# prosysscience/JSSEnv

Hardware: AMD Instinct MI355X
Metric: env steps/sec (batched) (higher is better)
Workload: dtype int32

## Files before the change

__graft_entry__.py:

```python
import os
import sys

ROOT = os.path.dirname(os.path.abspath(__file__))
if ROOT not in sys.path:
    sys.path.insert(0, ROOT)


def build() -> None:
    from jssenv_amd.build import build_cpu_twin, build_extension
    path = build_extension(force=True)
    assert os.path.isfile(path)
    twin = build_cpu_twin(force=True)
    assert os.path.isfile(twin)
    from oracle import build_oracle
    build_oracle(force=True)
    import ctypes
    from jssenv_amd import _abi
    _abi.bind_keys(_abi.bind_rules(_abi.bind_search(_abi.bind(ctypes.CDLL(path)))))
    _abi.bind_keys(_abi.bind_rules(_abi.bind_search(_abi.bind(ctypes.CDLL(twin)))))
    _abi.bind_bound(ctypes.CDLL(_abi.library_path("libjss_bound_hip.so")))
    _abi.bind_bound(ctypes.CDLL(twin))
    _abi.bind_order(ctypes.CDLL(_abi.library_path("libjss_order_hip.so")))
    _abi.bind_order(ctypes.CDLL(twin))
    _abi.bind_tabu(ctypes.CDLL(_abi.library_path("libjss_tabu_hip.so")))
    _abi.bind_tabu(ctypes.CDLL(twin))
    _abi.bind_block(ctypes.CDLL(_abi.library_path("libjss_block_hip.so")))
    _abi.bind_block(ctypes.CDLL(twin))
    _abi.bind_relink(ctypes.CDLL(_abi.library_path("libjss_relink_hip.so")))
    _abi.bind_relink(ctypes.CDLL(twin))
    _abi.bind_decode(ctypes.CDLL(_abi.library_path("libjss_decode_hip.so")))
    _abi.bind_decode(ctypes.CDLL(twin))
    _abi.bind_machine(ctypes.CDLL(_abi.library_path("libjss_machine_hip.so")))
    _abi.bind_machine(ctypes.CDLL(twin))
    _abi.bind_carlier(ctypes.CDLL(_abi.library_path("libjss_carlier_hip.so")))
    _abi.bind_carlier(ctypes.CDLL(twin))
    _abi.bind_propagate(ctypes.CDLL(_abi.library_path("libjss_propagate_hip.so")))
    _abi.bind_propagate(ctypes.CDLL(twin))
    import jssenv_amd
    print(f"built {path} and {twin}")


def smoke() -> None:
    import numpy as np
    import torch
    assert torch.cuda.is_available(), "smoke() needs a GPU"
    from jssenv_amd import BatchedJssEnv, builtin_instance
    from oracle import OracleEnv

    inst = builtin_instance("ta01")
    B, seed = 256, 3
    env = BatchedJssEnv(inst, batch=B, device="cuda:0", seed=seed)
    env.reset()
# ... 24 lines not shown
```

jssenv_amd/_abi.py:

```python
from __future__ import annotations

import ctypes as C
import os
from typing import Optional

ABI_VERSION = 14
STATE_LAYOUT = 7
MAX_JOBS, MAX_MACHINES = 128, 64
F_TODO, F_CUR, F_LEFT, F_PERF, F_IDLE, F_IDLE_LAST, F_F4, F_NEXT, NF = 0, 1, 2, 3, 4, 5, 6, 7, 8
TODO_MASK, FLAG_LEGAL, FLAG_BLOCKED, NEXT2_SHIFT = 255, 256, 512, 10
FC_W0, FC_LEFT_F4, FC_IDLE, FC_IDLE_LAST, NFC = 0, 1, 2, 3, 4
FC_TODO_MASK, FC_FLAG_LEGAL, FC_FLAG_BLOCKED, FC_FLAG_F4_ONE, FC_PERF_SHIFT = 127, 128, 256, 512, 10
FM_W0, FM_LEFT_F4, FM_PERF_NEXT, FM_NEXT_NEXT2, FM_IDLE, FM_IDLE_LAST, NFM = 0, 1, 2, 3, 4, 5, 6
FM_TODO_MASK, FM_FLAG_LEGAL, FM_FLAG_BLOCKED, FM_FLAG_F4_ONE, FM_CUR_SHIFT, FM_OP_MASK = 63, 64, 128, 256, 9, 0x1FFFFF
H_CLOCK, H_EPISODE, H_STEP, H_STATUS = 0, 1, 2, 3
NH = 4
C_JOBS, C_MACHINES, C_MAX_TIME_OP, C_TABLE, C_MAX_TIME_JOBS, C_SUM_OP = 0, 1, 2, 3, 4, 5
C_RCP_MAX_TIME_OP, C_RCP_MAX_TIME_JOBS, C_RCP_SUM_OP, C_RCP_MACHINES, NC = 6, 7, 8, 9, 12
STATUS_NOOP = 256
F4_ONE = -1
I_JOBS, I_MACHINES, I_MAX_TIME_OP, I_MAX_TIME_JOBS, I_SUM_OP = 0, 1, 2, 3, 4
I_RCP_MAX_TIME_OP, I_RCP_MAX_TIME_JOBS, I_RCP_SUM_OP, I_RCP_MACHINES, NI = 5, 6, 7, 8, 12
ERR_ILLEGAL_ACTION, ERR_NOPE_IDLE, ERR_BAD_ACTION, ERR_BAD_LOGITS, ERR_BAD_INDEX = 1, 2, 4, 8, 16
ACTION_SKIP, ACTION_RESET, ACTION_CLOSE = -1, -2, -3
# ... 78 lines not shown
MACHINE_SYMBOLS = ("jss_machine_relax", "jss_bottleneck_build")
BOTTLENECK_NI = 4
BOTTLENECK_MAX_REOPT = 8

CARLIER_VERSION = 1
CARLIER_SYMBOLS = ("jss_machine_solve", "jss_bottleneck_exact")
CARLIER_MAX_NODES = 4096
CARLIER_MAX_DEPTH = 64
EXACT_NI = 8

PROPAGATE_VERSION = 1
PROPAGATE_SYMBOLS = ("jss_propagate",)
PROPAGATE_MAX_PASSES = 4096
PROPAGATE_MAX_TIME = 0x3FFFFFFF
PROPAGATE_FIXPOINT, PROPAGATE_REFUTED, PROPAGATE_BUDGET = 0, 1, 2

_p = C.c_void_p


class JssDesc(C.Structure):
    _fields_ = [("batch", C.c_int32), ("jmax", C.c_int32), ("mmax", C.c_int32), ("n_tables", C.c_int32),
                ("ops", _p), ("rem", _p), ("inst", _p), ("table_of_env", _p), ("env_ids", _p),
                ("env_id_base", C.c_int64), ("kernel", C.c_int32), ("threads", C.c_int32),
                ("jmin", C.c_int32), ("record_ints", C.c_int32), ("cr_factor", C.c_double),
                ("jclass", C.c_int32), ("mclass", C.c_int32)]


class JssState(C.Structure):
    _fields_ = [("env", _p), ("env_const", _p), ("job", _p), ("machine", _p), ("solution", _p), ("counters", _p)]

# ... 315 lines not shown
    symbols, binder, header = _FAMILIES[family]
    first = getattr(lib, symbols[0], None)
    if first is not None and first.argtypes is not None:
        return lib
    if not all(hasattr(lib, name) for name in symbols):
        if what is None:
            return None
        raise RuntimeError(f"{what}: the loaded library does not export the {family}_* calls of include/{header}")
    return binder(lib)


def check(lib, rc: int, what: str):
    if rc != 0:
        msg = lib.jss_error_string(rc)
        raise RuntimeError(f"{what} failed: {rc} ({msg.decode() if msg else '?'})")
```

jssenv_amd/backends.py:

```python
from __future__ import annotations

import ctypes as C
import os

import numpy as np

from . import _abi


class HipBackend:

    name = "hip"
    default_kernel = "auto"

    def __init__(self, device=None):
        import torch
        if not torch.cuda.is_available():
            raise RuntimeError("jssenv_amd needs an AMD GPU (torch.cuda.is_available() is False); there is no silent "
                               "CPU fallback -- pass device='cpu' to run on the host-core twin (libjss_cpu.so) on purpose")
        path = _abi.library_path()
        if not os.path.isfile(path):
            raise RuntimeError(f"{path} is missing: build it with `python -c 'import __graft_entry__ as g; g.build()'`")
        self.torch = torch
        self.device = torch.device(device if device is not None else f"cuda:{torch.cuda.current_device()}")
# ... 7 lines not shown
        if not self.lib.jss_backend().startswith(b"hip"):
            raise RuntimeError(f"{path} is not the HIP library ({self.lib.jss_backend()!r})")
        self._scalars = {}
        self._stream_arrays = {}
        self._raw_stream = getattr(torch._C, "_cuda_getCurrentRawStream", None)
        self._beam_lib = None
        self._bound_lib = None
        self._order_lib = None
        self._tabu_lib = None
        self._block_lib = None
        self._relink_lib = None
        self._decode_lib = None
        self._machine_lib = None
        self._carlier_lib = None
        self._propagate_lib = None

    @property
    def beam_lib(self):
        if self._beam_lib is None:
            path = _abi.library_path("libjss_beam_hip.so")
            if not os.path.isfile(path):
                raise RuntimeError(f"{path} is missing: build it with `python -c 'import __graft_entry__ as g; g.build()'`")
            self._beam_lib = _abi.bind_beam(C.CDLL(path))
        return self._beam_lib

    @property
    def bound_lib(self):
        if self._bound_lib is None:
            path = _abi.library_path("libjss_bound_hip.so")
            if not os.path.isfile(path):
# ... 345 lines not shown
```

jssenv_amd/build.py:

```python
import os
import shutil
import subprocess

_HERE = os.path.dirname(os.path.abspath(__file__))
_ROOT = os.path.dirname(_HERE)
SRC = os.path.join(_HERE, "csrc", "jss_kernels.hip")
OUT = os.path.join(_HERE, "libjss_hip.so")
FLAGS = ["--offload-arch=gfx950", "-O3", "-std=c++17", "-fPIC", "-shared", "-I" + os.path.join(_ROOT, "include"),
         "-mllvm", "-amdgpu-atomic-optimizer-strategy=None"]
CPU_SRC = os.path.join(_HERE, "csrc", "jss_cpu.cpp")
CPU_OUT = os.path.join(_HERE, "libjss_cpu.so")
CPU_FLAGS = ["-O3", "-std=c++17", "-fopenmp", "-fPIC", "-shared", "-Wall", "-I" + os.path.join(_ROOT, "include")]
_HEADER = os.path.join(_ROOT, "include", "jss_hip.h")
_SEARCH = os.path.join(_ROOT, "include", "jss_search.h")
_RULES = os.path.join(_ROOT, "include", "jss_rules.h")
_KEYS = os.path.join(_ROOT, "include", "jss_keys.h")
_BEAM = os.path.join(_ROOT, "include", "jss_beam.h")
BEAM_SRC = os.path.join(_HERE, "csrc", "jss_beam.hip")
BEAM_OUT = os.path.join(_HERE, "libjss_beam_hip.so")
_BOUND = os.path.join(_ROOT, "include", "jss_bound.h")
BOUND_SRC = os.path.join(_HERE, "csrc", "jss_bound.hip")
BOUND_OUT = os.path.join(_HERE, "libjss_bound_hip.so")
_ORDER = os.path.join(_ROOT, "include", "jss_order.h")
ORDER_SRC = os.path.join(_HERE, "csrc", "jss_order.hip")
# ... 7 lines not shown
_RELINK = os.path.join(_ROOT, "include", "jss_relink.h")
RELINK_SRC = os.path.join(_HERE, "csrc", "jss_relink.hip")
RELINK_OUT = os.path.join(_HERE, "libjss_relink_hip.so")
_DECODE = os.path.join(_ROOT, "include", "jss_decode.h")
DECODE_SRC = os.path.join(_HERE, "csrc", "jss_decode.hip")
DECODE_OUT = os.path.join(_HERE, "libjss_decode_hip.so")
_MACHINE = os.path.join(_ROOT, "include", "jss_machine.h")
MACHINE_SRC = os.path.join(_HERE, "csrc", "jss_machine.hip")
MACHINE_OUT = os.path.join(_HERE, "libjss_machine_hip.so")
_CARLIER = os.path.join(_ROOT, "include", "jss_carlier.h")
CARLIER_SRC = os.path.join(_HERE, "csrc", "jss_carlier.hip")
CARLIER_OUT = os.path.join(_HERE, "libjss_carlier_hip.so")
_PROPAGATE = os.path.join(_ROOT, "include", "jss_propagate.h")
PROPAGATE_SRC = os.path.join(_HERE, "csrc", "jss_propagate.hip")
PROPAGATE_OUT = os.path.join(_HERE, "libjss_propagate_hip.so")
_OWN_LIBRARY = (os.path.basename(BEAM_SRC), os.path.basename(BOUND_SRC), os.path.basename(ORDER_SRC),
                os.path.basename(TABU_SRC), os.path.basename(BLOCK_SRC), os.path.basename(RELINK_SRC),
                os.path.basename(DECODE_SRC), os.path.basename(MACHINE_SRC), os.path.basename(CARLIER_SRC), os.path.basename(PROPAGATE_SRC))
_CHECKS = os.path.join(_HERE, "csrc", "jss_abi_checks.hpp")
_ROWS = os.path.join(_HERE, "csrc", "jss_env_rows.hpp")


def hipcc() -> str:
    for cand in (shutil.which("hipcc"), "/opt/rocm/bin/hipcc"):
        if cand and os.path.isfile(cand):
            return cand
    raise RuntimeError("hipcc not found")


def _fresh(out, deps):
    return os.path.isfile(out) and all(os.path.getmtime(out) >= os.path.getmtime(d) for d in deps)


def build_extension(force: bool = False, extra=(), out: str = OUT) -> str:
    csrc = os.path.dirname(SRC)
    deps = [os.path.join(csrc, f) for f in os.listdir(csrc) if f.endswith((".hip", ".hpp")) and f not in _OWN_LIBRARY] + [_HEADER, _SEARCH, _RULES, _KEYS, _BEAM, _BOUND, _ORDER, _TABU, _BLOCK, _RELINK, _DECODE, _MACHINE, _CARLIER, _PROPAGATE]
    if out == OUT:
        build_beam_extension(force)
        build_bound_extension(force)
        build_order_extension(force)
        build_tabu_extension(force)
        build_block_extension(force)
        build_relink_extension(force)
        build_decode_extension(force)
        build_machine_extension(force)
        build_carlier_extension(force)
        build_propagate_extension(force)
    if not force and _fresh(out, deps):
        return out
    subprocess.check_call([hipcc(), *FLAGS, *extra, SRC, "-o", out])
    return out


def build_beam_extension(force: bool = False) -> str:
    if not force and _fresh(BEAM_OUT, [BEAM_SRC, _CHECKS, _HEADER, _SEARCH, _RULES, _KEYS, _BEAM, _BOUND, _ORDER, _TABU, _BLOCK, _RELINK, _DECODE, _MACHINE, _CARLIER, _PROPAGATE]):
        return BEAM_OUT
    tmp = BEAM_OUT + f".tmp{os.getpid()}"
    subprocess.check_call([hipcc(), *FLAGS, BEAM_SRC, "-o", tmp])
    os.replace(tmp, BEAM_OUT)
    return BEAM_OUT


# ... 64 lines not shown
    if not force and _fresh(CARLIER_OUT, [CARLIER_SRC, _CHECKS, _HEADER, _SEARCH, _RULES, _KEYS, _BEAM, _BOUND, _ORDER, _TABU, _BLOCK, _RELINK, _DECODE, _MACHINE, _CARLIER, _PROPAGATE]):
        return CARLIER_OUT
    tmp = CARLIER_OUT + f".tmp{os.getpid()}"
    subprocess.check_call([hipcc(), *FLAGS, CARLIER_SRC, "-o", tmp])
    os.replace(tmp, CARLIER_OUT)
    return CARLIER_OUT


def build_propagate_extension(force: bool = False) -> str:
    if not force and _fresh(PROPAGATE_OUT, [PROPAGATE_SRC, _CHECKS, _HEADER, _SEARCH, _RULES, _KEYS, _BEAM, _BOUND, _ORDER, _TABU, _BLOCK, _RELINK, _DECODE, _MACHINE, _CARLIER, _PROPAGATE]):
        return PROPAGATE_OUT
    tmp = PROPAGATE_OUT + f".tmp{os.getpid()}"
    subprocess.check_call([hipcc(), *FLAGS, PROPAGATE_SRC, "-o", tmp])
    os.replace(tmp, PROPAGATE_OUT)
    return PROPAGATE_OUT


def build_cpu_twin(force: bool = False) -> str:
    if not force and _fresh(CPU_OUT, [CPU_SRC, _CHECKS, _ROWS, _HEADER, _SEARCH, _RULES, _KEYS, _BEAM, _BOUND, _ORDER, _TABU, _BLOCK, _RELINK, _DECODE, _MACHINE, _CARLIER, _PROPAGATE]):
        return CPU_OUT
    cxx = shutil.which("g++") or shutil.which("c++")
    if not cxx:
        raise RuntimeError("g++ not found")
    tmp = CPU_OUT + f".tmp{os.getpid()}"
    subprocess.check_call([cxx, *CPU_FLAGS, CPU_SRC, "-o", tmp])
    os.replace(tmp, CPU_OUT)
    return CPU_OUT
```

jssenv_amd/csrc/jss_packed_env.hpp:

```cpp
#pragma once
#include "jss_common.hpp"

namespace jss {

template <class T>
__device__ __forceinline__ T ld_off(const void *base, unsigned byte_off) {
    return *reinterpret_cast<const T *>(reinterpret_cast<const char *>(base) + byte_off);
}
template <class T>
__device__ __forceinline__ void st_off(void *base, unsigned byte_off, T v) {
    *reinterpret_cast<T *>(reinterpret_cast<char *>(base) + byte_off) = v;
}
typedef float jss_v4f __attribute__((vector_size(16)));
__device__ __forceinline__ void st_nt(void *base, unsigned byte_off, float4 v) {
    const jss_v4f x = {v.x, v.y, v.z, v.w};
    __builtin_nontemporal_store(x, reinterpret_cast<jss_v4f *>(reinterpret_cast<char *>(base) + byte_off));
}

template <bool WT, class T>
__device__ __forceinline__ void st_out(void *base, unsigned byte_off, T v) {
    if (WT) wt_store(reinterpret_cast<T *>(reinterpret_cast<char *>(base) + byte_off), v);
    else st_off<T>(base, byte_off, v);
}

template <int G, int TAB>
struct PCtx {
    int lane, gl, gbase;
    unsigned rel;
    int first_env;
    bool alive;
    bool jvalid, mvalid;
    int tid;
    int J, M, max_time_op;
    int max_time_jobs, sum_op;
    float r_op, r_jobs, r_sum, r_m;
    int32_t *norm;
    const int32_t *lds_row;
// ... 685 lines not shown
                         (int)((unsigned)e.left | ((unsigned)(one ? 0 : e.f4) << 16)),
                         (int)((unsigned)e.perf | (nxt << 21)), (int)((nxt >> 11) | (nxt2 << 10)));
        r.hi = make_int4(e.idle, e.idle_last, 0, 0);
    } else {
        r.lo = make_int4(e.todo | (e.legal ? JSS_FLAG_LEGAL : 0) | (e.blocked ? JSS_FLAG_BLOCKED : 0) |
                             (e.nxt2 >= 0 ? (int)((unsigned)e.nxt2 << JSS_NEXT2_SHIFT) : 0), e.cur, e.left, e.perf);
        r.hi = make_int4(e.idle, e.idle_last, e.f4, e.nxt);
    }
    return r;
}

enum { kStoreAll = 0, kStoreCompare = 1, kStoreCause = 2 };
#ifndef JSS_ONE_STEP_STORES
#define JSS_ONE_STEP_STORES kStoreCause
#endif
template <int G, int TAB, int DIFF = kStoreCompare>
__device__ __forceinline__ void p_store(const PEnv<G> &e, const PCtx<G, TAB> &c, const Params &p, const PHeader &hd,
                                        const PRaw<G> &raw, bool fresh, bool moved = false, int a_sched = -1) {
    if (!c.alive) return;
    const bool adv = DIFF == kStoreCause && moved;
    const unsigned jm = (unsigned)p.d.jmax, mm = (unsigned)p.d.mmax;
    const size_t fe = (size_t)c.first_env;
    const PRaw<G> now = p_pack(e, c, hd);
    if (c.gl == 0) {
        st_off(p.s.env + fe * JSS_NH, c.rel * (JSS_NH * 4u), now.h);
        if (fresh) {
            const PNorm n = p_norm(c);
            int32_t *cp = p.s.env_const + fe * JSS_NC;
            const unsigned co = c.rel * (JSS_NC * 4u);
            st_off(cp, co, make_int4(c.J, c.M, c.max_time_op, c.tid));
            st_off(cp, co + 16u, make_int4(n.max_time_jobs, n.sum_op, as_int(n.r_op), as_int(n.r_jobs)));
            st_off(cp, co + 32u, make_int4(as_int(n.r_sum), as_int(n.r_m), 0, 0));
        }
    }
    if (tab_no_clocks(TAB)) {
    } else if (fresh ? (unsigned)c.gl < mm : (c.mvalid && (DIFF == kStoreAll || e.tm != raw.tm)))
        st_off(p.s.machine + fe * mm, (c.rel * mm + c.gl) * 4u, e.tm);
    const bool w0_changed = now.lo.x != raw.lo.x;
    const bool head_dirty = w0_changed || c.gl == a_sched || (adv && e.cur >= 0);
    const bool rest_dirty = adv && (e.cur >= 0 || w0_changed);
// ... 8 lines not shown
                    st_off(jb, jo + 8u, make_int2(lo.z, lo.w));
                    st_off(jb, jo + 16u, make_int2(hi.x, hi.y));
                }
            } else {
                if (DIFF == kStoreAll || fresh || lo.x != raw.lo.x || lo.y != raw.lo.y) st_off(jb, jo, make_int2(lo.x, lo.y));
                if (DIFF == kStoreAll || fresh || lo.z != raw.lo.z || lo.w != raw.lo.w) st_off(jb, jo + 8u, make_int2(lo.z, lo.w));
                if (DIFF == kStoreAll || fresh || hi.x != raw.hi.x || hi.y != raw.hi.y) st_off(jb, jo + 16u, make_int2(hi.x, hi.y));
            }
        }
    } else if (tab_compact(TAB)) {
        if (c.jvalid || (fresh && (unsigned)c.gl < jm)) {
            const int4 lo = now.lo;
            bool dirty;
            if (DIFF == kStoreCause) dirty = head_dirty || rest_dirty;
            else dirty = DIFF == kStoreAll || lo.x != raw.lo.x || lo.y != raw.lo.y || lo.z != raw.lo.z || lo.w != raw.lo.w;
            if (fresh || dirty) st_off(p.s.job + fe * jm * JSS_NFC, (c.rel * jm + c.gl) * (JSS_NFC * 4u), lo);
        }
    } else if (c.jvalid || (fresh && (unsigned)c.gl < jm)) {
        int32_t *jb = p.s.job + fe * jm * JSS_NF;
        const unsigned jo = (c.rel * jm + c.gl) * 32u;
        const int4 lo = now.lo, hi = now.hi;
        if (DIFF == kStoreCause && !fresh) {
            if (head_dirty) st_off(jb, jo, lo);
            if (rest_dirty) st_off(jb, jo + 16u, hi);
        } else {
            if (DIFF == kStoreAll || fresh || lo.x != raw.lo.x || lo.y != raw.lo.y || lo.z != raw.lo.z || lo.w != raw.lo.w) st_off(jb, jo, lo);
            if (DIFF == kStoreAll || fresh || hi.x != raw.hi.x || hi.y != raw.hi.y || hi.z != raw.hi.z || hi.w != raw.hi.w) st_off(jb, jo + 16u, hi);
        }
        if (fresh)
            for (unsigned r = (unsigned)c.gl + G; r < jm; r += G) {
                st_off(jb, (c.rel * jm + r) * 32u, make_int4(0, -1, 0, 0));
// ... 107 lines not shown
        st_out<WT, uint8_t>(p.o.done + fe, c.rel, (uint8_t)(r.done ? 1 : 0));
        if (r.done) st_out<WT, int>(p.o.makespan + fe, c.rel * 4u, e.t);
        if (p.s.counters) add_counters(p.s.counters + (fe + c.rel) * 4, 1, r.done ? 1 : 0, r.done ? e.t : 0, r.rn);
    }
}
template <int G, int TAB, bool WT>
__device__ __forceinline__ bool p_step_call(PEnv<G> &e, PHeader &hd, PCtx<G, TAB> &c, const Params &p, int a_in,
                                            int32_t *mvtab, int &rn, bool &called) {
    const PStepResult r = p_step_compute<G, TAB, WT>(e, hd, c, p, a_in, mvtab);
    p_step_outputs<G, TAB, WT>(e, c, p, r);
    rn = r.rn;
    called = r.called;
    return r.restart;
}

template <int G, int MODE, int TAB>
__device__ __forceinline__ bool p_body(PEnv<G> &e, PHeader &hd, PCtx<G, TAB> &c, const Params &p, int a_in, bool selected,
                                       int32_t *mvtab, float *scratch, bool wave_whole, int &a_sched, bool &restarted, int cw = 0) {
    const size_t fe = (size_t)c.first_env;
    bool fresh = false;
    a_sched = -1;
    restarted = false;
    if (MODE == kReset) {
        const bool on = c.alive && selected;
        p_reset(e, c, p, on);
        if (on) {
            fresh = true;
            hd.episode += 1;
            hd.step = 0;
            if (c.gl == 0) {
                st_off<float>(p.o.reward + fe, c.rel * 4u, 0.f);
// ... 36 lines not shown
        const uint64_t env_id = (uint64_t)(p.d.env_ids ? ld_off<int64_t>(p.d.env_ids + fe, c.rel * 8u)
                                                       : p.d.env_id_base + (int64_t)(fe + c.rel));
        int n_steps = 0, n_done = 0, last_rn = 0, last_makespan = -1, sum_makespan = 0, sum_rn = 0;
        const bool autoreset = (p.flags & JSS_ROLLOUT_AUTORESET) != 0;
        const int n_iter = MODE == kRollout1 ? 1 : p.n_iter;
        for (int it = 0; it < n_iter; ++it) {
            const size_t slot0 = (size_t)it * traj_stride(p) + fe;
            if (MODE == kTraj) {
                if (p.t.real_obs) p_store_obs<G, TAB>(e, c, p, p.t.real_obs + slot0 * p.d.jmax * 7, scratch, wave_whole);
                if (p.t.action_mask) p_store_mask<G, TAB>(e, c, p, p.t.action_mask + slot0 * (p.d.jmax + 1));
            }
            const bool done0 = !grp_any<G>(e.legal, c.gbase);
            const bool do_reset = c.alive && done0 && autoreset;
            const bool do_step = c.alive && !done0;
            if (MODE != kRollout1 && MODE != kTraj && __ballot(do_reset || do_step) == 0) break;
            p_reset(e, c, p, do_reset);
            if (do_reset) {
                hd.episode += 1;
                hd.step = 0;
            }
            int a = JSS_ABLATED(p, JSS_ABLATE_SELECT) ? __ffs(grp_ballot<G>(e.legal, c.gbase)) - 1
                                                      : p_select<G, TAB, false, rule_source(MODE, TAB)>(e, c, p, env_id, (uint32_t)hd.episode, (uint32_t)hd.step);
            if (!do_step) a = JSS_ACTION_SKIP;
            if (MODE == kRollout1) {
                a_sched = a;
                restarted = do_reset;
            }
            const int rn = p_step(e, c, p, a, mvtab);
            const bool done1 = !grp_any<G>(e.legal, c.gbase);
            if (do_step) {
                last_rn = rn;
                hd.step += 1;
                n_steps += 1;
                sum_rn += rn;
                if (done1) {
                    n_done += 1;
                    sum_makespan += e.t;
                    last_makespan = e.t;
                }
            }
            if (MODE == kTraj && c.alive && c.gl == 0) {
                const size_t slot = slot0 + c.rel;
                if (p.t.action) p.t.action[slot] = do_step ? a : (do_reset ? JSS_ACTION_RESET : JSS_ACTION_SKIP);
                if (p.t.reward) p.t.reward[slot] = do_step ? div_by((float)rn, (float)c.max_time_op, p_norm(c).r_op) : 0.f;
                if (p.t.done) p.t.done[slot] = do_step ? (done1 ? 1 : 0) : (do_reset ? 0 : 1);
            }
        }
        const bool done = !grp_any<G>(e.legal, c.gbase);
#ifdef JSS_COUNTERS_PLAIN
        if (p.s.counters) p_bump_counters(c, p, cw, n_steps, n_done, sum_makespan, sum_rn);
#endif
        if (c.alive && c.gl == 0) {
            if (n_steps) st_off<float>(p.o.reward + fe, c.rel * 4u, div_by((float)last_rn, (float)c.max_time_op, p_norm(c).r_op));
            st_off<uint8_t>(p.o.done + fe, c.rel, done ? 1 : 0);
            if (last_makespan >= 0) st_off<int>(p.o.makespan + fe, c.rel * 4u, last_makespan);
#ifndef JSS_COUNTERS_PLAIN
            if (p.s.counters) add_counters(p.s.counters + (fe + c.rel) * 4, n_steps, n_done, sum_makespan, sum_rn);
#endif
        }
    }
    return fresh;
}

__device__ __forceinline__ void p_lookahead_score(const Params &p, int cand, int makespan, int steps, int reward_num) {
    p.la.makespan[cand] = makespan;
    if (p.la.steps) p.la.steps[cand] = steps;
    if (p.la.reward_num) p.la.reward_num[cand] = reward_num;
}
template <int G, int TAB>
__device__ __forceinline__ void p_lookahead(PEnv<G> &e, PHeader &hd, const PCtx<G, TAB> &c, const Params &p, int cand,
// ... 28 lines not shown
    if (cand_alive && c.gl == 0) p_lookahead_score(p, cand, ok && done ? e.t : -1, ok ? n_steps : 0, ok ? sum_rn : 0);
}

#ifndef JSS_PTRAJ_LDS_MIN_BLOCKS
#define JSS_PTRAJ_LDS_MIN_BLOCKS 5
#endif
#ifndef JSS_PTRAJ_GLOBAL_MIN_BLOCKS
#define JSS_PTRAJ_GLOBAL_MIN_BLOCKS 4
#endif
#ifndef JSS_PACKED_GLOBAL_MIN_BLOCKS
#define JSS_PACKED_GLOBAL_MIN_BLOCKS 7
#endif
#ifndef JSS_PACKED_MEDIUM_MIN_BLOCKS
#define JSS_PACKED_MEDIUM_MIN_BLOCKS 8
#endif
template <int G, int MODE, int TAB, bool PADDED = false>
__device__ __forceinline__ void packed_block(const Params &p, int block, int32_t *lds) {
    static_assert(!PADDED || (MODE != kTraj && MODE != kSteps && MODE != kSession), "the recorders write whole rows");
    constexpr int E = kWave / G;
    constexpr int EB = E * kWavesPerBlock;
    const int lane = threadIdx.x & (kWave - 1);
    const int wave = __builtin_amdgcn_readfirstlane((int)(threadIdx.x >> 6));
    if constexpr (rule_source(MODE, TAB) == kRwLds) {
        if (threadIdx.x == 0) rule_stash_put(p.keys);
    }
    float *scratch = reinterpret_cast<float *>(lds + p.table_lds_ints) + wave * p.obs_wave_floats;
    int32_t *mvtab = lds + p.mv_off_ints + wave * kWave;

    PCtx<G, TAB> c;
    c.lane = lane;
    c.gl = lane & (G - 1);
    c.gbase = lane & ~(G - 1);
    c.norm = lds + p.norm_off_ints + wave * kWave + c.gbase;
// ... 80 lines not shown
    c.jvalid = c.gl < c.J;
    c.mvalid = c.gl < c.M;
    c.lds_row = lds + (c.gl < p.d.jmax ? c.gl : 0) * p.d.mmax;

    PEnv<G> e;
    PHeader hd = p_unpack(e, c, raw, mvtab);
    if (MODE != kReset && hd.episode == 0) c.alive = false;
    if constexpr (MODE == kLookahead) {
        p_lookahead(e, hd, c, p, cand, cand_alive, a_la, mvtab);
        return;
    }
    if constexpr (MODE == kLogits) a_in = p_logits_pick(e, c, p, (uint32_t)hd.episode, (uint32_t)hd.step, a_in, lr);
    int a_sched;
    bool restarted;
#ifdef JSS_COUNTERS_PLAIN
    const bool fresh = p_body<G, MODE, TAB>(e, hd, c, p, a_in, selected, mvtab, scratch, wave_whole, a_sched, restarted, raw.cw);
#else
    const bool fresh = p_body<G, MODE, TAB>(e, hd, c, p, a_in, selected, mvtab, scratch, wave_whole, a_sched, restarted);
#endif
    if (MODE == kPolicy) return;
    constexpr int kDiffStores = (MODE == kRollout || MODE == kTraj || MODE == kSteps) ? kStoreAll
                                : ((MODE == kStep || MODE == kLogits || MODE == kRollout1) && tab_global(TAB)) ? JSS_ONE_STEP_STORES : kStoreCompare;
    p_store<G, TAB, kDiffStores>(e, c, p, hd, raw, fresh, restarted || e.t != raw.h.x, a_sched);
    p_store_mask<G, TAB, false, PADDED>(e, c, p, p.o.action_mask + fe * (p.d.jmax + 1));
    if (!JSS_ABLATED(p, JSS_ABLATE_OBS))
        p_store_obs<G, TAB, false, PADDED>(e, c, p, p.o.real_obs + fe * p.d.jmax * 7, scratch, wave_whole);
}

template <int G, int MODE, int TAB>
__global__ __launch_bounds__(kBlock, (MODE == kTraj || MODE == kSteps) ? (tab_global(TAB) && !tab_medium(TAB) ? JSS_PTRAJ_GLOBAL_MIN_BLOCKS : JSS_PTRAJ_LDS_MIN_BLOCKS)
                                     : (MODE == kRollout || MODE == kLookahead) ? (tab_global(TAB) ? 4 : 5)
                                     : (tab_medium(TAB) && MODE == kRollout1) ? JSS_PACKED_MEDIUM_MIN_BLOCKS
                                     : ((tab_global(TAB) && (MODE == kStep || MODE == kLogits || MODE == kRollout1)) ? JSS_PACKED_GLOBAL_MIN_BLOCKS : 8))
void jss_packed_kernel(Params p_arg) {
    HIP_DYNAMIC_SHARED(int32_t, lds)
    JSS_PARAMS_OF(p, p_arg, (MODE == kTraj || MODE == kSteps || MODE == kRollout || MODE == kLookahead) && (tab_global(TAB) || MODE == kTraj));
    packed_block<G, MODE, TAB>(p, (int)blockIdx.x, lds);
}


template <int TAB>
// ... 226 lines not shown
```

jssenv_amd/env.py:

```python
from __future__ import annotations

import ctypes as C
import os
from typing import Optional, Sequence, Union

import numpy as np

from . import _abi
from .backends import _NULL_CTX, CpuBackend, HipBackend, _carve_numpy, make_backend
from .instances import Instance, PackedBatch, MAX_DURATION, OP_MACHINE_SHIFT, pack_batch, resolve_instance


class _Selector:
    __slots__ = ("arg", "keep", "family", "stock")

    def __init__(self, arg, keep=None, family="jss"):
        self.stock = family == "jss"
        self.arg, self.keep, self.family = arg if self.stock else C.byref(arg), (arg, keep), family

    def call(self, lib, verb, head, *tail):
        name = self.family + "_" + verb
        rc = getattr(lib, name)(*head, self.arg, *tail)
        if rc:
            _abi.check(lib, rc, name)
# ... 1454 lines not shown
    def _logits_struct(self, arg, temperature, logp, entropy, first=0):
        ptr, row, dtype, _ = arg
        item = 2 if dtype == _abi.LOGITS_BF16 else 4
        at = lambda t, on: self._row_ptr(t, first) if on else None
        return _abi.JssLogits(ptr + first * row * item, row, dtype, float(temperature), at(self._lg_action, True),
                              at(self._lg_logp, logp), at(self._lg_entropy, entropy))

    def _logits_info(self, logp, entropy):
        info = {"action": self._lg_action}
        if logp:
            info["logp"] = self._lg_logp
        if entropy:
            info["entropy"] = self._lg_entropy
        return info

    def rollout(self, kind: Union[str, int] = "random", n_iter: int = 1, seed: Optional[int] = None,
                autoreset: bool = True, explore: float = 0.0, weights=None, keys=None, nope_key=None):
        if not self._is_reset:
            raise RuntimeError("call reset() before rollout()")
        be = self.backend
        sel = self._selector(kind, "rollout", weights, keys, nope_key)
        n_iter, flags = int(n_iter), _abi.ROLLOUT_AUTORESET if autoreset else 0
        d, s, o = self._refs()
        if autoreset and self.fresh:
            if not sel.stock:
                self._refuse_fresh(f"rollout(kind='{kind}', autoreset=True)")
            if n_iter > 1:
                self._refuse_fresh("rollout(n_iter > 1, autoreset=True)")
            self.generate(self.done)
        sd, q16 = self.seed if seed is None else int(seed), int(round(explore * 65536))
        if not sel.stock or self._classes is None:
            with be.on_device():
                sel.call(be.lib, "rollout", (d, s, o), sd, q16, n_iter, flags, be.stream())
        elif n_iter == 1:
            with be.on_device():
                streams = (C.c_void_p * 1)(be.stream())
                rc = be.lib.jss_multi_rollout(self._classes["n"], *self._classes["sets"], sel.arg, sd, q16, 1, flags, 1, streams)
                _abi.check(be.lib, rc, "jss_multi_rollout")
        else:
            self._over_ranges(lambda dk, sk, ok, _a, stream: be.lib.jss_rollout(dk, sk, ok, sel.arg, sd, q16, n_iter, flags, stream),
                              "jss_rollout")
        return self._obs(), self.reward, self.done, False, {}

    def rollout_steps(self, kind: Union[str, int] = "random", steps: int = 1, n_sub: int = 2, seed: Optional[int] = None,
                      autoreset: bool = True, explore: float = 0.0):
        if not self._is_reset:
# ... 3 lines not shown
        if not 1 <= int(n_sub) <= _abi.MAX_SUB_BATCHES:
            raise ValueError(f"n_sub must be in [1, {_abi.MAX_SUB_BATCHES}]")
        be = self.backend
        k = stock_code(kind, "rollout_steps")
        flags = _abi.ROLLOUT_AUTORESET if autoreset else 0
        d, s, o = self._refs()
        sd = self.seed if seed is None else int(seed)
        with be.on_device():
            if self._classes is not None:
                n = min(int(n_sub), 4)
                streams = be.stream_array(n) if hasattr(be, "stream_array") else (C.c_void_p * n)()
                rc = be.lib.jss_multi_rollout(self._classes["n"], *self._classes["sets"], k, sd, int(round(explore * 65536)), int(steps),
                                              flags | (_abi.ROLLOUT_FORK_JOIN if n > 1 and hasattr(be, "stream_array") else 0), n, streams)
                _abi.check(be.lib, rc, "jss_multi_rollout")
                return self._obs(), self.reward, self.done, False, {}
            if hasattr(be, "stream_array"):
                rc = be.lib.jss_rollout_steps(d, s, o, k, sd, int(round(explore * 65536)), int(steps),
                                              flags | _abi.ROLLOUT_FORK_JOIN, int(n_sub), be.stream_array(int(n_sub)))
            else:
                rc = be.with_streams(int(n_sub), lambda streams: be.lib.jss_rollout_steps(
                    d, s, o, k, sd, int(round(explore * 65536)), int(steps), flags, int(n_sub), streams), self._stream_events)
        _abi.check(be.lib, rc, "jss_rollout_steps")
        return self._obs(), self.reward, self.done, False, {}

    def policy_step_steps(self, kind: Union[str, int] = "random", steps: int = 1, n_sub: int = 2, seed: Optional[int] = None,
                          autoreset: bool = True, explore: float = 0.0, caller_orders_streams: bool = False):
        if not self._is_reset:
            raise RuntimeError("call reset() before policy_step_steps()")
        if autoreset:
            self._refuse_fresh("policy_step_steps(autoreset=True)")
        if not 1 <= int(n_sub) <= _abi.MAX_SUB_BATCHES:
            raise ValueError(f"n_sub must be in [1, {_abi.MAX_SUB_BATCHES}]")
        be = self.backend
        k = stock_code(kind, "policy_step_steps")
        flags = (_abi.ROLLOUT_AUTORESET if autoreset else 0)
# ... 12 lines not shown

    def bind_rollout_steps(self, kind: Union[str, int] = "random", steps: int = 1, n_sub: int = 2, seed: Optional[int] = None,
                           autoreset: bool = True, explore: float = 0.0, caller_orders_streams: bool = False):
        if not self._is_reset:
            raise RuntimeError("call reset() before rollout_steps()")
        if autoreset:
            self._refuse_fresh("rollout_steps(autoreset=True)")
        be = self.backend
        if not hasattr(be, "stream_array"):
            return lambda: self.rollout_steps(kind, steps, n_sub, seed, autoreset, explore)
        k = stock_code(kind, "bind_rollout_steps")
        flags = (_abi.ROLLOUT_AUTORESET if autoreset else 0) | (0 if caller_orders_streams else _abi.ROLLOUT_FORK_JOIN)
        d, s, o = self._refs()
        with be.on_device():
            streams = be.stream_array(int(n_sub))
        fn, sd, q16, n_steps, n = be.lib.jss_rollout_steps, self.seed if seed is None else int(seed), int(round(explore * 65536)), int(steps), int(n_sub)
        lib = be.lib
        if self._classes is not None:
            n = min(n, 4)
            with be.on_device():
                streams = be.stream_array(n)
            if n == 1:
                flags &= ~_abi.ROLLOUT_FORK_JOIN
            n_sets, sets, fm = self._classes["n"], self._classes["sets"], be.lib.jss_multi_rollout

            def issue_classes():
                rc = fm(n_sets, *sets, k, sd, q16, n_steps, flags, n, streams)
                if rc:
                    _abi.check(lib, rc, "jss_multi_rollout")
            return issue_classes

# ... 416 lines not shown
```

Before: 4.860 billion.

## Add dedicated one-step rollout library with write-through stores for compact records

Adds a separate HIP library whose kernel runs a single rollout step per launch for single-table compact-record instances up to 32x32. Its state, mask and observation stores are write-through, and the Python rollout and rollout_steps paths route to it by default. The aim is to cut cache pollution or write-back cost on the per-step stores and to use a specialised kernel build. The cost is another library to build and bind, plus a different store path that may interact badly with the existing diff-store logic.

```diff
diff --git a/__graft_entry__.py b/__graft_entry__.py
--- a/__graft_entry__.py
+++ b/__graft_entry__.py
@@ -36,6 +36,7 @@
     _abi.bind_carlier(ctypes.CDLL(twin))
     _abi.bind_propagate(ctypes.CDLL(_abi.library_path("libjss_propagate_hip.so")))
     _abi.bind_propagate(ctypes.CDLL(twin))
+    _abi.bind_onestep(ctypes.CDLL(_abi.library_path("libjss_onestep_hip.so")))
     import jssenv_amd
     print(f"built {path} and {twin}")
 
diff --git a/include/jss_onestep.h b/include/jss_onestep.h
--- /dev/null
+++ b/include/jss_onestep.h
@@ -0,0 +1,23 @@
+#ifndef JSS_ONESTEP_H
+#define JSS_ONESTEP_H
+
+#include "jss_hip.h"
+
+#ifdef __cplusplus
+extern "C" {
+#endif
+
+#define JSS_ONESTEP_VERSION 1
+
+int jss_onestep_version(void);
+
+int jss_onestep_rollout(const JssDesc *desc, const JssState *state, const JssOut *out, int kind, uint64_t seed,
+                        uint32_t explore_q16, int32_t n_iter, int32_t flags, void *stream);
+
+int jss_onestep_rollout_steps(const JssDesc *desc, const JssState *state, const JssOut *out, int kind, uint64_t seed,
+                              uint32_t explore_q16, int32_t n_steps, int32_t flags, int32_t n_sub, void *const *streams);
+
+#ifdef __cplusplus
+}
+#endif
+#endif
diff --git a/jssenv_amd/_abi.py b/jssenv_amd/_abi.py
--- a/jssenv_amd/_abi.py
+++ b/jssenv_amd/_abi.py
@@ -116,6 +116,10 @@
 PROPAGATE_MAX_PASSES = 4096
 PROPAGATE_MAX_TIME = 0x3FFFFFFF
 PROPAGATE_FIXPOINT, PROPAGATE_REFUTED, PROPAGATE_BUDGET = 0, 1, 2
+
+ONESTEP_VERSION = 1
+ONESTEP_SYMBOLS = ("jss_onestep_version", "jss_onestep_rollout", "jss_onestep_rollout_steps")
+ONESTEP_MAX_GROUP = 32
 
 _p = C.c_void_p
 
@@ -461,3 +465,20 @@
     if rc != 0:
         msg = lib.jss_error_string(rc)
         raise RuntimeError(f"{what} failed: {rc} ({msg.decode() if msg else '?'})")
+
+
+def bind_onestep(lib):
+    for name in ONESTEP_SYMBOLS:
+        if not hasattr(lib, name):
+            raise AttributeError(f"library does not export {name}")
+    D, S, O = C.POINTER(JssDesc), C.POINTER(JssState), C.POINTER(JssOut)
+    lib.jss_onestep_version.restype = C.c_int
+    lib.jss_onestep_version.argtypes = []
+    lib.jss_onestep_rollout.restype = C.c_int
+    lib.jss_onestep_rollout.argtypes = [D, S, O, C.c_int, C.c_uint64, C.c_uint32, C.c_int32, C.c_int32, _p]
+    lib.jss_onestep_rollout_steps.restype = C.c_int
+    lib.jss_onestep_rollout_steps.argtypes = [D, S, O, C.c_int, C.c_uint64, C.c_uint32, C.c_int32, C.c_int32, C.c_int32,
+                                              C.POINTER(_p)]
+    if lib.jss_onestep_version() != ONESTEP_VERSION:
+        raise RuntimeError(f"include/jss_onestep.h version {lib.jss_onestep_version()}, this package binds {ONESTEP_VERSION}")
+    return lib
diff --git a/jssenv_amd/backends.py b/jssenv_amd/backends.py
--- a/jssenv_amd/backends.py
+++ b/jssenv_amd/backends.py
@@ -45,6 +45,16 @@
         self._machine_lib = None
         self._carlier_lib = None
         self._propagate_lib = None
+        self._onestep_lib = None
+
+    @property
+    def onestep_lib(self):
+        if self._onestep_lib is None:
+            path = _abi.library_path("libjss_onestep_hip.so")
+            if not os.path.isfile(path):
+                raise RuntimeError(f"{path} is missing: build it (jssenv_amd.build.build_onestep_extension)")
+            self._onestep_lib = _abi.bind_onestep(C.CDLL(path))
+        return self._onestep_lib
 
     @property
     def beam_lib(self):
diff --git a/jssenv_amd/build.py b/jssenv_amd/build.py
--- a/jssenv_amd/build.py
+++ b/jssenv_amd/build.py
@@ -45,9 +45,13 @@
 _PROPAGATE = os.path.join(_ROOT, "include", "jss_propagate.h")
 PROPAGATE_SRC = os.path.join(_HERE, "csrc", "jss_propagate.hip")
 PROPAGATE_OUT = os.path.join(_HERE, "libjss_propagate_hip.so")
+_ONESTEP = os.path.join(_ROOT, "include", "jss_onestep.h")
+ONESTEP_SRC = os.path.join(_HERE, "csrc", "jss_onestep.hip")
+ONESTEP_OUT = os.path.join(_HERE, "libjss_onestep_hip.so")
 _OWN_LIBRARY = (os.path.basename(BEAM_SRC), os.path.basename(BOUND_SRC), os.path.basename(ORDER_SRC),
                 os.path.basename(TABU_SRC), os.path.basename(BLOCK_SRC), os.path.basename(RELINK_SRC),
-                os.path.basename(DECODE_SRC), os.path.basename(MACHINE_SRC), os.path.basename(CARLIER_SRC), os.path.basename(PROPAGATE_SRC))
+                os.path.basename(DECODE_SRC), os.path.basename(MACHINE_SRC), os.path.basename(CARLIER_SRC), os.path.basename(PROPAGATE_SRC),
+                os.path.basename(ONESTEP_SRC))
 _CHECKS = os.path.join(_HERE, "csrc", "jss_abi_checks.hpp")
 _ROWS = os.path.join(_HERE, "csrc", "jss_env_rows.hpp")
 
@@ -77,6 +81,7 @@
         build_machine_extension(force)
         build_carlier_extension(force)
         build_propagate_extension(force)
+        build_onestep_extension(force)
     if not force and _fresh(out, deps):
         return out
     subprocess.check_call([hipcc(), *FLAGS, *extra, SRC, "-o", out])
@@ -171,6 +176,18 @@
     subprocess.check_call([hipcc(), *FLAGS, PROPAGATE_SRC, "-o", tmp])
     os.replace(tmp, PROPAGATE_OUT)
     return PROPAGATE_OUT
+
+
+def build_onestep_extension(force: bool = False, extra=(), out: str = ONESTEP_OUT) -> str:
+    csrc = os.path.dirname(ONESTEP_SRC)
+    deps = [ONESTEP_SRC, _CHECKS, _ROWS, _ONESTEP, _HEADER, _SEARCH, _RULES, _KEYS] + \
+           [os.path.join(csrc, f) for f in ("jss_common.hpp", "jss_packed_env.hpp")]
+    if not force and _fresh(out, deps):
+        return out
+    tmp = out + f".tmp{os.getpid()}"
+    subprocess.check_call([hipcc(), *FLAGS, *extra, ONESTEP_SRC, "-o", tmp])
+    os.replace(tmp, out)
+    return out
 
 
 def build_cpu_twin(force: bool = False) -> str:
diff --git a/jssenv_amd/csrc/jss_onestep.hip b/jssenv_amd/csrc/jss_onestep.hip
--- /dev/null
+++ b/jssenv_amd/csrc/jss_onestep.hip
@@ -0,0 +1,170 @@
+#include <mutex>
+#include <unordered_map>
+
+#include "jss_common.hpp"
+#include "jss_packed_env.hpp"
+#include "jss_abi_checks.hpp"
+#include "jss_env_rows.hpp"
+#include "jss_onestep.h"
+
+namespace jss {
+
+template <int G>
+__global__ __launch_bounds__(kBlock, 8) void jss_onestep_kernel(Params p_arg) {
+    HIP_DYNAMIC_SHARED(int32_t, lds)
+    JSS_PARAMS_OF(p, p_arg, false);
+    packed_block<G, kRollout1, kTabLdsC, false, true>(p, (int)blockIdx.x, lds);
+}
+
+}
+
+namespace {
+using namespace jss;
+using namespace jss_abi;
+
+constexpr size_t kMaxDynamicLds = 64 * 1024;
+
+struct ForkJoinEvents {
+    hipEvent_t fork = nullptr;
+    hipEvent_t join[16] = {};
+};
+std::mutex g_events_mutex;
+std::unordered_map<void *, ForkJoinEvents> g_events;
+
+int events_for(void *main_stream, ForkJoinEvents **out) {
+    std::lock_guard<std::mutex> lock(g_events_mutex);
+    ForkJoinEvents &ev = g_events[main_stream];
+    if (!ev.fork) {
+        if (hipEventCreateWithFlags(&ev.fork, hipEventDisableTiming) != hipSuccess) return (int)hipGetLastError();
+        for (int i = 0; i < 16; ++i)
+            if (hipEventCreateWithFlags(&ev.join[i], hipEventDisableTiming) != hipSuccess) return (int)hipGetLastError();
+    }
+    *out = &ev;
+    return 0;
+}
+
+int fork_streams(const ForkJoinEvents &ev, void *const *streams, int n) {
+    if (hipEventRecord(ev.fork, reinterpret_cast<hipStream_t>(streams[0])) != hipSuccess) return (int)hipGetLastError();
+    for (int i = 1; i < n; ++i)
+        if (hipStreamWaitEvent(reinterpret_cast<hipStream_t>(streams[i]), ev.fork, 0) != hipSuccess) return (int)hipGetLastError();
+    return 0;
+}
+int join_streams(const ForkJoinEvents &ev, void *const *streams, int n) {
+    int rc = 0;
+    for (int i = 1; i < n; ++i) {
+        if (hipEventRecord(ev.join[i], reinterpret_cast<hipStream_t>(streams[i])) != hipSuccess ||
+            hipStreamWaitEvent(reinterpret_cast<hipStream_t>(streams[0]), ev.join[i], 0) != hipSuccess) {
+            const int e = (int)hipGetLastError();
+            if (!rc) rc = e;
+        }
+    }
+    return rc;
+}
+
+int check_class(const JssDesc *d) {
+    if (d->n_tables != 1 || d->table_of_env) return JSS_E_SHAPE;
+    if (d->record_ints != JSS_NFC) return JSS_E_SHAPE;
+    if (d->jmax > 32 || d->mmax > 32) return JSS_E_SHAPE;
+    if (d->kernel & JSS_KERNEL_WAVE) return JSS_E_KIND;
+    return 0;
+}
+
+struct Plan {
+    void (*fn)(Params);
+    int envs_per_block;
+    size_t shmem;
+};
+
+int plan(Params &p, Plan &lp) {
+    const int G = p.d.jmax <= 16 && p.d.mmax <= 16 ? 16 : 32;
+    p.region_ints = p.d.jmax * p.d.mmax;
+    p.table_lds_ints = (p.region_ints + 3) & ~3;
+    p.obs_wave_floats = ((kWave / G) * p.d.jmax * 7 + 3) & ~3;
+    p.mv_off_ints = p.table_lds_ints + kWavesPerBlock * p.obs_wave_floats;
+    p.norm_off_ints = p.mv_off_ints + kBlock;
+    lp.shmem = sizeof(int32_t) * (size_t)p.norm_off_ints;
+    if (lp.shmem > kMaxDynamicLds) return JSS_E_LDS;
+    lp.envs_per_block = (kWave / G) * kWavesPerBlock;
+    lp.fn = G == 16 ? jss_onestep_kernel<16> : jss_onestep_kernel<32>;
+    return 0;
+}
+
+int fire(const Params &p, const Plan &lp, void *stream) {
+    if (p.d.batch == 0) return 0;
+    const int blocks = (p.d.batch + lp.envs_per_block - 1) / lp.envs_per_block;
+    hipLaunchKernelGGL(lp.fn, dim3(blocks), dim3(kBlock), lp.shmem, reinterpret_cast<hipStream_t>(stream), p);
+    return (int)hipGetLastError();
+}
+
+Params params_of(const JssDesc *desc, const JssState *state, const JssOut *out, int kind, uint64_t seed, uint32_t explore_q16,
+                 int32_t flags) {
+    Params p = {};
+    p.d = *desc;
+    p.s = *state;
+    p.o = *out;
+    p.kind = kind; p.seed = seed; p.explore_q16 = explore_q16;
+    p.n_iter = 1; p.flags = flags & ~JSS_ROLLOUT_FORK_JOIN;
+    return p;
+}
+
+Params sub_batch(const Params &p, int start, int count) {
+    Params q = p;
+    const size_t s0 = (size_t)start;
+    q.d.batch = count;
+    if (p.d.env_ids) q.d.env_ids = p.d.env_ids + s0;
+    q.d.env_id_base = p.d.env_id_base + start;
+    for_each_env_row(p.d, q.s, q.o, [s0](auto *&rows, size_t bytes, bool) {
+        if (rows) rows = reinterpret_cast<decltype(+rows)>(reinterpret_cast<char *>(rows) + s0 * bytes);
+    });
+    return q;
+}
+
+struct Part {
+    int start, count;
+};
+int cut(int batch, int n_sub, Part *parts) {
+    const int chunk = (((batch + n_sub - 1) / n_sub) + 63) & ~63;
+    int n = 0;
+    for (int start = 0; n < n_sub && start < batch; start += chunk) parts[n++] = Part{start, batch - start < chunk ? batch - start : chunk};
+    return n;
+}
+
+}
+
+extern "C" {
+
+int jss_onestep_version(void) { return JSS_ONESTEP_VERSION; }
+
+int jss_onestep_rollout(const JssDesc *desc, const JssState *state, const JssOut *out, int kind, uint64_t seed,
+                        uint32_t explore_q16, int32_t n_iter, int32_t flags, void *stream) {
+    int rc = check_rollout(desc, state, out, stock_selector(kind), n_iter);
+    if (rc || (rc = check_class(desc))) return rc;
+    if (n_iter != 1) return JSS_E_SHAPE;
+    Params p = params_of(desc, state, out, kind, seed, explore_q16, flags);
+    Plan lp;
+    if ((rc = plan(p, lp))) return rc;
+    return fire(p, lp, stream);
+}
+
+int jss_onestep_rollout_steps(const JssDesc *desc, const JssState *state, const JssOut *out, int kind, uint64_t seed,
+                              uint32_t explore_q16, int32_t n_steps, int32_t flags, int32_t n_sub, void *const *streams) {
+    int rc = check_rollout_steps(desc, state, out, kind, n_steps, n_sub, streams);
+    if (rc || (rc = check_class(desc))) return rc;
+    if (n_steps == 0) return 0;
+    Params p = params_of(desc, state, out, kind, seed, explore_q16, flags);
+    Plan lp;
+    if ((rc = plan(p, lp))) return rc;
+    Part parts[16];
+    Params sub[16];
+    const int n = cut(desc->batch, n_sub, parts);
+    for (int i = 0; i < n; ++i) sub[i] = sub_batch(p, parts[i].start, parts[i].count);
+    const bool fork_join = (flags & JSS_ROLLOUT_FORK_JOIN) != 0 && n > 1;
+    ForkJoinEvents *ev = nullptr;
+    if (fork_join && ((rc = events_for(streams[0], &ev)) || (rc = fork_streams(*ev, streams, n)))) return rc;
+    for (int s = 0; s < n_steps && !rc; ++s)
+        for (int i = 0; i < n && !rc; ++i) rc = fire(sub[i], lp, streams[i]);
+    const int jrc = fork_join ? join_streams(*ev, streams, n) : 0;
+    return rc ? rc : jrc;
+}
+
+}
diff --git a/jssenv_amd/csrc/jss_packed_env.hpp b/jssenv_amd/csrc/jss_packed_env.hpp
--- a/jssenv_amd/csrc/jss_packed_env.hpp
+++ b/jssenv_amd/csrc/jss_packed_env.hpp
@@ -21,6 +21,17 @@
 __device__ __forceinline__ void st_out(void *base, unsigned byte_off, T v) {
     if (WT) wt_store(reinterpret_cast<T *>(reinterpret_cast<char *>(base) + byte_off), v);
     else st_off<T>(base, byte_off, v);
+}
+
+template <bool WT>
+__device__ __forceinline__ void st_out16(void *base, unsigned byte_off, int4 v) {
+    if (WT) {
+        float4 f;
+        f.x = as_float(v.x); f.y = as_float(v.y); f.z = as_float(v.z); f.w = as_float(v.w);
+        wt_store16(base, byte_off, f);
+    } else {
+        st_off(base, byte_off, v);
+    }
 }
 
 template <int G, int TAB>
@@ -736,16 +747,17 @@
 #ifndef JSS_ONE_STEP_STORES
 #define JSS_ONE_STEP_STORES kStoreCause
 #endif
-template <int G, int TAB, int DIFF = kStoreCompare>
+template <int G, int TAB, int DIFF = kStoreCompare, bool WT = false>
 __device__ __forceinline__ void p_store(const PEnv<G> &e, const PCtx<G, TAB> &c, const Params &p, const PHeader &hd,
                                         const PRaw<G> &raw, bool fresh, bool moved = false, int a_sched = -1) {
+    static_assert(!WT || tab_compact(TAB), "write-through state stores: compact records only");
     if (!c.alive) return;
     const bool adv = DIFF == kStoreCause && moved;
     const unsigned jm = (unsigned)p.d.jmax, mm = (unsigned)p.d.mmax;
     const size_t fe = (size_t)c.first_env;
     const PRaw<G> now = p_pack(e, c, hd);
     if (c.gl == 0) {
-        st_off(p.s.env + fe * JSS_NH, c.rel * (JSS_NH * 4u), now.h);
+        st_out16<WT>(p.s.env + fe * JSS_NH, c.rel * (JSS_NH * 4u), now.h);
         if (fresh) {
             const PNorm n = p_norm(c);
             int32_t *cp = p.s.env_const + fe * JSS_NC;
@@ -784,7 +796,7 @@
             bool dirty;
             if (DIFF == kStoreCause) dirty = head_dirty || rest_dirty;
             else dirty = DIFF == kStoreAll || lo.x != raw.lo.x || lo.y != raw.lo.y || lo.z != raw.lo.z || lo.w != raw.lo.w;
-            if (fresh || dirty) st_off(p.s.job + fe * jm * JSS_NFC, (c.rel * jm + c.gl) * (JSS_NFC * 4u), lo);
+            if (fresh || dirty) st_out16<WT>(p.s.job + fe * jm * JSS_NFC, (c.rel * jm + c.gl) * (JSS_NFC * 4u), lo);
         }
     } else if (c.jvalid || (fresh && (unsigned)c.gl < jm)) {
         int32_t *jb = p.s.job + fe * jm * JSS_NF;
@@ -922,7 +934,7 @@
     return r.restart;
 }
 
-template <int G, int MODE, int TAB>
+template <int G, int MODE, int TAB, bool WT = false>
 __device__ __forceinline__ bool p_body(PEnv<G> &e, PHeader &hd, PCtx<G, TAB> &c, const Params &p, int a_in, bool selected,
                                        int32_t *mvtab, float *scratch, bool wave_whole, int &a_sched, bool &restarted, int cw = 0) {
     const size_t fe = (size_t)c.first_env;
@@ -989,7 +1001,7 @@
             const bool do_reset = c.alive && done0 && autoreset;
             const bool do_step = c.alive && !done0;
             if (MODE != kRollout1 && MODE != kTraj && __ballot(do_reset || do_step) == 0) break;
-            p_reset(e, c, p, do_reset);
+            p_reset<G, TAB, WT>(e, c, p, do_reset);
             if (do_reset) {
                 hd.episode += 1;
                 hd.step = 0;
@@ -1001,7 +1013,7 @@
                 a_sched = a;
                 restarted = do_reset;
             }
-            const int rn = p_step(e, c, p, a, mvtab);
+            const int rn = p_step<G, TAB, WT>(e, c, p, a, mvtab);
             const bool done1 = !grp_any<G>(e.legal, c.gbase);
             if (do_step) {
                 last_rn = rn;
@@ -1026,9 +1038,9 @@
         if (p.s.counters) p_bump_counters(c, p, cw, n_steps, n_done, sum_makespan, sum_rn);
 #endif
         if (c.alive && c.gl == 0) {
-            if (n_steps) st_off<float>(p.o.reward + fe, c.rel * 4u, div_by((float)last_rn, (float)c.max_time_op, p_norm(c).r_op));
-            st_off<uint8_t>(p.o.done + fe, c.rel, done ? 1 : 0);
-            if (last_makespan >= 0) st_off<int>(p.o.makespan + fe, c.rel * 4u, last_makespan);
+            if (n_steps) st_out<WT, float>(p.o.reward + fe, c.rel * 4u, div_by((float)last_rn, (float)c.max_time_op, p_norm(c).r_op));
+            st_out<WT, uint8_t>(p.o.done + fe, c.rel, (uint8_t)(done ? 1 : 0));
+            if (last_makespan >= 0) st_out<WT, int>(p.o.makespan + fe, c.rel * 4u, last_makespan);
 #ifndef JSS_COUNTERS_PLAIN
             if (p.s.counters) add_counters(p.s.counters + (fe + c.rel) * 4, n_steps, n_done, sum_makespan, sum_rn);
 #endif
@@ -1087,9 +1099,10 @@
 #ifndef JSS_PACKED_MEDIUM_MIN_BLOCKS
 #define JSS_PACKED_MEDIUM_MIN_BLOCKS 8
 #endif
-template <int G, int MODE, int TAB, bool PADDED = false>
+template <int G, int MODE, int TAB, bool PADDED = false, bool WT = false>
 __device__ __forceinline__ void packed_block(const Params &p, int block, int32_t *lds) {
     static_assert(!PADDED || (MODE != kTraj && MODE != kSteps && MODE != kSession), "the recorders write whole rows");
+    static_assert(!WT || (MODE == kRollout1 && tab_compact(TAB) && !PADDED), "write-through stores: p_body's rollout branch, compact records");
     constexpr int E = kWave / G;
     constexpr int EB = E * kWavesPerBlock;
     const int lane = threadIdx.x & (kWave - 1);
@@ -1200,17 +1213,17 @@
     int a_sched;
     bool restarted;
 #ifdef JSS_COUNTERS_PLAIN
-    const bool fresh = p_body<G, MODE, TAB>(e, hd, c, p, a_in, selected, mvtab, scratch, wave_whole, a_sched, restarted, raw.cw);
+    const bool fresh = p_body<G, MODE, TAB, WT>(e, hd, c, p, a_in, selected, mvtab, scratch, wave_whole, a_sched, restarted, raw.cw);
 #else
-    const bool fresh = p_body<G, MODE, TAB>(e, hd, c, p, a_in, selected, mvtab, scratch, wave_whole, a_sched, restarted);
+    const bool fresh = p_body<G, MODE, TAB, WT>(e, hd, c, p, a_in, selected, mvtab, scratch, wave_whole, a_sched, restarted);
 #endif
     if (MODE == kPolicy) return;
     constexpr int kDiffStores = (MODE == kRollout || MODE == kTraj || MODE == kSteps) ? kStoreAll
                                 : ((MODE == kStep || MODE == kLogits || MODE == kRollout1) && tab_global(TAB)) ? JSS_ONE_STEP_STORES : kStoreCompare;
-    p_store<G, TAB, kDiffStores>(e, c, p, hd, raw, fresh, restarted || e.t != raw.h.x, a_sched);
-    p_store_mask<G, TAB, false, PADDED>(e, c, p, p.o.action_mask + fe * (p.d.jmax + 1));
+    p_store<G, TAB, kDiffStores, WT>(e, c, p, hd, raw, fresh, restarted || e.t != raw.h.x, a_sched);
+    p_store_mask<G, TAB, WT, PADDED>(e, c, p, p.o.action_mask + fe * (p.d.jmax + 1));
     if (!JSS_ABLATED(p, JSS_ABLATE_OBS))
-        p_store_obs<G, TAB, false, PADDED>(e, c, p, p.o.real_obs + fe * p.d.jmax * 7, scratch, wave_whole);
+        p_store_obs<G, TAB, WT, PADDED>(e, c, p, p.o.real_obs + fe * p.d.jmax * 7, scratch, wave_whole);
 }
 
 template <int G, int MODE, int TAB>
diff --git a/jssenv_amd/env.py b/jssenv_amd/env.py
--- a/jssenv_amd/env.py
+++ b/jssenv_amd/env.py
@@ -1492,6 +1492,18 @@
             info["entropy"] = self._lg_entropy
         return info
 
+    def _onestep_lib(self, kind_code):
+        be = self.backend
+        in_class = self.__dict__.get("_onestep_class")
+        if in_class is None:
+            d = self._desc
+            in_class = self._onestep_class = bool(
+                hasattr(be, "onestep_lib") and self._classes is None and d.n_tables == 1 and not d.table_of_env
+                and d.record_ints == _abi.NFC and not (d.kernel & 1) and max(d.jmax, d.mmax) <= _abi.ONESTEP_MAX_GROUP)
+        if not in_class or not 0 <= kind_code < (1 << 24) or os.environ.get("JSS_ONESTEP", "1") == "0":
+            return None
+        return be.onestep_lib
+
     def rollout(self, kind: Union[str, int] = "random", n_iter: int = 1, seed: Optional[int] = None,
                 autoreset: bool = True, explore: float = 0.0, weights=None, keys=None, nope_key=None):
         if not self._is_reset:
@@ -1507,7 +1519,11 @@
                 self._refuse_fresh("rollout(n_iter > 1, autoreset=True)")
             self.generate(self.done)
         sd, q16 = self.seed if seed is None else int(seed), int(round(explore * 65536))
-        if not sel.stock or self._classes is None:
+        one = self._onestep_lib(sel.arg) if sel.stock and n_iter == 1 else None
+        if one is not None:
+            with be.on_device():
+                _abi.check(be.lib, one.jss_onestep_rollout(d, s, o, sel.arg, sd, q16, 1, flags, be.stream()), "jss_onestep_rollout")
+        elif not sel.stock or self._classes is None:
             with be.on_device():
                 sel.call(be.lib, "rollout", (d, s, o), sd, q16, n_iter, flags, be.stream())
         elif n_iter == 1:
@@ -1541,11 +1557,13 @@
                                               flags | (_abi.ROLLOUT_FORK_JOIN if n > 1 and hasattr(be, "stream_array") else 0), n, streams)
                 _abi.check(be.lib, rc, "jss_multi_rollout")
                 return self._obs(), self.reward, self.done, False, {}
+            one = self._onestep_lib(k)
+            fn = be.lib.jss_rollout_steps if one is None else one.jss_onestep_rollout_steps
             if hasattr(be, "stream_array"):
-                rc = be.lib.jss_rollout_steps(d, s, o, k, sd, int(round(explore * 65536)), int(steps),
-                                              flags | _abi.ROLLOUT_FORK_JOIN, int(n_sub), be.stream_array(int(n_sub)))
+                rc = fn(d, s, o, k, sd, int(round(explore * 65536)), int(steps),
+                        flags | _abi.ROLLOUT_FORK_JOIN, int(n_sub), be.stream_array(int(n_sub)))
             else:
-                rc = be.with_streams(int(n_sub), lambda streams: be.lib.jss_rollout_steps(
+                rc = be.with_streams(int(n_sub), lambda streams: fn(
                     d, s, o, k, sd, int(round(explore * 65536)), int(steps), flags, int(n_sub), streams), self._stream_events)
         _abi.check(be.lib, rc, "jss_rollout_steps")
         return self._obs(), self.reward, self.done, False, {}
@@ -1588,7 +1606,9 @@
         d, s, o = self._refs()
         with be.on_device():
             streams = be.stream_array(int(n_sub))
-        fn, sd, q16, n_steps, n = be.lib.jss_rollout_steps, self.seed if seed is None else int(seed), int(round(explore * 65536)), int(steps), int(n_sub)
+        one = self._onestep_lib(k)
+        fn = be.lib.jss_rollout_steps if one is None else one.jss_onestep_rollout_steps
+        sd, q16, n_steps, n = self.seed if seed is None else int(seed), int(round(explore * 65536)), int(steps), int(n_sub)
         lib = be.lib
         if self._classes is not None:
             n = min(n, 4)
```

Measured after the change: 5.099 billion, median of 6. +4.9%, better.
